# lijx10/DeepI2P

Measured on NVIDIA B200. Metric: registrations/sec, higher is better.
Workload: dtype f64

## Files before the change

deepi2p_b200/csrc/frustum_solver.cu:

```cuda
#include <cfloat>
#include <cmath>
#include <cstdarg>
#include <cstdlib>

#include "common.cuh"

namespace dib {

static thread_local char g_err[512] = "";
void set_error(const char* fmt, ...) {
  va_list ap;
  va_start(ap, fmt);
  vsnprintf(g_err, sizeof(g_err), fmt, ap);
  va_end(ap);
}

#ifndef DIB_WARPS_F4
#define DIB_WARPS_F4 10
#endif
#ifndef DIB_WARPS_F6
#define DIB_WARPS_F6 7
#endif
#ifndef DIB_WARPS_D4
#define DIB_WARPS_D4 7
#endif
#ifndef DIB_WARPS_D6
#define DIB_WARPS_D6 5
#endif
#ifndef DIB_CTAS_PER_SM
#define DIB_CTAS_PER_SM 2
#endif
template <typename CT, int P> struct Cfg;
template <> struct Cfg<float, 4> { static constexpr int kWarps = DIB_WARPS_F4; };
template <> struct Cfg<float, 6> { static constexpr int kWarps = DIB_WARPS_F6; };
template <> struct Cfg<double, 4> { static constexpr int kWarps = DIB_WARPS_D4; };
template <> struct Cfg<double, 6> { static constexpr int kWarps = DIB_WARPS_D6; };

struct Cam {
  double fx, fy, cx, cy, W1, H1, hW, hH;
};

struct PoseConst {
  double R[9];
  double t[3];
  double Jl[9];
  double cD, sD;
  int small;
};

template <int P>
struct NAcc {
  static constexpr int NA = P * (P + 1) / 2;
  static constexpr int N = 1 + P + NA;
};

__host__ __device__ constexpr int tri(int P, int j, int k) {
  return j * P - j * (j - 1) / 2 + (k - j);
}


template <int P>
__device__ __noinline__ void make_pose(const double* x, PoseConst* pc) {
  if (P == 4) {
    const double ry = x[0];
    pc->t[0] = x[1]; pc->t[1] = x[2]; pc->t[2] = x[3];
    double c, s;
    if (ry * ry > DBL_EPSILON) { sincos(ry, &s, &c); pc->cD = c; pc->sD = s; pc->small = 0; }
    else { c = 1.0; s = ry; pc->cD = 1.0; pc->sD = 0.0; pc->small = 1; }
    pc->R[0] = c; pc->R[1] = 0; pc->R[2] = s;
    pc->R[3] = 0; pc->R[4] = 1; pc->R[5] = 0;
    pc->R[6] = -s; pc->R[7] = 0; pc->R[8] = c;
  } else {
    const double ax = x[0], ay = x[1], az = x[2];
    pc->t[0] = x[3]; pc->t[1] = x[4]; pc->t[2] = x[5];
    const double th2 = ax * ax + ay * ay + az * az;
    if (th2 > DBL_EPSILON) {
      const double th = sqrt(th2);
      double s, c;
      sincos(th, &s, &c);
      const double wx = ax / th, wy = ay / th, wz = az / th;
      const double omc = 1.0 - c;
      pc->R[0] = c + wx * wx * omc;      pc->R[1] = wx * wy * omc - wz * s; pc->R[2] = wy * s + wx * wz * omc;
      pc->R[3] = wz * s + wx * wy * omc; pc->R[4] = c + wy * wy * omc;      pc->R[5] = -wx * s + wy * wz * omc;
      pc->R[6] = -wy * s + wx * wz * omc; pc->R[7] = wx * s + wy * wz * omc; pc->R[8] = c + wz * wz * omc;
      double sh, ch;
      sincos(0.5 * th, &sh, &ch);
      const double q = sh / (0.5 * th);
      const double A = 0.5 * q * q;
      double B;
      if (th < 0.5) {
        const double t2 = th2;
        B = 1.0 / 6.0 + t2 * (-1.0 / 120.0 + t2 * (1.0 / 5040.0 + t2 * (-1.0 / 362880.0 +
            t2 * (1.0 / 39916800.0 + t2 * (-1.0 / 6227020800.0 + t2 * (1.0 / 1307674368000.0))))));
      } else {
        B = (th - s) / (th2 * th);
      }
      pc->Jl[0] = 1.0 + B * (ax * ax - th2); pc->Jl[1] = -A * az + B * ax * ay;     pc->Jl[2] = A * ay + B * ax * az;
      pc->Jl[3] = A * az + B * ax * ay;      pc->Jl[4] = 1.0 + B * (ay * ay - th2); pc->Jl[5] = -A * ax + B * ay * az;
      pc->Jl[6] = -A * ay + B * ax * az;     pc->Jl[7] = A * ax + B * ay * az;      pc->Jl[8] = 1.0 + B * (az * az - th2);
      pc->small = 0;
    } else {
      pc->R[0] = 1;   pc->R[1] = -az; pc->R[2] = ay;
      pc->R[3] = az;  pc->R[4] = 1;   pc->R[5] = -ax;
      pc->R[6] = -ay; pc->R[7] = ax;  pc->R[8] = 1;
      for (int i = 0; i < 9; ++i) pc->Jl[i] = (i % 4 == 0) ? 1.0 : 0.0;
      pc->small = 1;
    }
    pc->cD = 0; pc->sD = 0;
  }
}

struct SmemAcc {
  double* base;
  __device__ __forceinline__ double& operator[](int j) const { return base[j * 32]; }
};

template <int P, typename ACC>
__device__ __forceinline__ void rank1(ACC acc, const double* J, double w, double r) {
  const double wr = w * r;
#pragma unroll
  for (int j = 0; j < P; ++j) {
    acc[1 + j] = fma(wr, J[j], acc[1 + j]);
    const double wj = w * J[j];
#pragma unroll
    for (int k = j; k < P; ++k) acc[1 + P + tri(P, j, k)] = fma(wj, J[k], acc[1 + P + tri(P, j, k)]);
  }
}

template <int P>
__device__ __forceinline__ bool point_rows(double px, double py, double pz, int lab, const Cam& cam,
                                           const PoseConst& pc, double r[3], double J[3][P], int* nrows) {
  constexpr int NR = P - 3;
  const double rx = fma(pc.R[0], px, fma(pc.R[1], py, pc.R[2] * pz));
  const double ry_ = fma(pc.R[3], px, fma(pc.R[4], py, pc.R[5] * pz));
  const double rz = fma(pc.R[6], px, fma(pc.R[7], py, pc.R[8] * pz));
  const double X = rx + pc.t[0], Y = ry_ + pc.t[1], Z = rz + pc.t[2];
  const double iz = 1.0 / Z;
  const double u = fma(cam.fx * X, iz, cam.cx);
  const double v = fma(cam.fy * Y, iz, cam.cy);

  bool any = false;
  double su = 0.0, sv = 0.0, sz = 0.0;
  if (lab == 0) {
    *nrows = 1;
    const double du_ = u - cam.hW, dv_ = v - cam.hH;
    const double xd = cam.hW - fabs(du_);
    const double yd = cam.hH - fabs(dv_);
    r[0] = 0.0;
    if (Z > 0.0 && xd > 0.0 && yd > 0.0) {
      r[0] = xd + yd;
      su = (du_ < 0.0) ? 1.0 : -1.0;
      sv = (dv_ < 0.0) ? 1.0 : -1.0;
      any = true;
    }
  } else {
    *nrows = 3;
    const double a0 = -u, b0 = u - cam.W1;
    const double a1 = -v, b1 = v - cam.H1;
    r[0] = (a0 < 0.0 ? 0.0 : a0) + (b0 < 0.0 ? 0.0 : b0);
    r[1] = (a1 < 0.0 ? 0.0 : a1) + (b1 < 0.0 ? 0.0 : b1);
    r[2] = (-Z < 0.0 ? 0.0 : -Z) * 100.0;
    su = (a0 < 0.0 ? 0.0 : -1.0) + (b0 < 0.0 ? 0.0 : 1.0);
    sv = (a1 < 0.0 ? 0.0 : -1.0) + (b1 < 0.0 ? 0.0 : 1.0);
    sz = (-Z < 0.0) ? 0.0 : -100.0;
    any = (su != 0.0) || (sv != 0.0) || (sz != 0.0);
  }
  if (!any) return false;

  double dX[NR], dY[NR], dZ[NR];
  if (P == 4) {
    dX[0] = fma(-pc.sD, px, pc.cD * pz);
    dY[0] = 0.0;
    dZ[0] = -fma(pc.cD, px, pc.sD * pz);
  } else {
    const double a = pc.small ? px : rx, b = pc.small ? py : ry_, c = pc.small ? pz : rz;
#pragma unroll
    for (int k = 0; k < 3; ++k) {
      dX[k] = c * pc.Jl[3 + k] - b * pc.Jl[6 + k];
      dY[k] = a * pc.Jl[6 + k] - c * pc.Jl[k];
      dZ[k] = b * pc.Jl[k] - a * pc.Jl[3 + k];
    }
  }
  const double au = cam.fx * iz, bu = (u - cam.cx) * iz;
  const double av = cam.fy * iz, bv = (v - cam.cy) * iz;
  double dU[P], dV[P];
#pragma unroll
  for (int k = 0; k < NR; ++k) {
    dU[k] = au * dX[k] - bu * dZ[k];
    dV[k] = av * dY[k] - bv * dZ[k];
  }
  dU[NR] = au; dU[NR + 1] = 0.0; dU[NR + 2] = -bu;
  dV[NR] = 0.0; dV[NR + 1] = av; dV[NR + 2] = -bv;
  if (lab == 0) {
#pragma unroll
    for (int j = 0; j < P; ++j) J[0][j] = su * dU[j] + sv * dV[j];
  } else {
#pragma unroll
    for (int j = 0; j < P; ++j) { J[0][j] = su * dU[j]; J[1][j] = sv * dV[j]; }
#pragma unroll
    for (int k = 0; k < NR; ++k) J[2][k] = sz * dZ[k];
    J[2][NR] = 0.0; J[2][NR + 1] = 0.0; J[2][NR + 2] = sz;
  }
  return true;
}

template <int P>
struct Proj {
  double X, Y, Z, iz, u, v;
  double dX[P - 3], dY[P - 3], dZ[P - 3];
};

template <int P>
__device__ __forceinline__ void project_point(double px, double py, double pz, bool valid, const Cam& cam,
                                              const PoseConst& pc, Proj<P>& o) {
  constexpr int NR = P - 3;
  if (!valid) { px = 0.0; py = 0.0; pz = 0.0; }
  double rx, ry_, rz;
  if (P == 4) {
    rx = fma(pc.R[0], px, pc.R[2] * pz);
    ry_ = py;
    rz = fma(pc.R[6], px, pc.R[8] * pz);
  } else {
    rx = fma(pc.R[0], px, fma(pc.R[1], py, pc.R[2] * pz));
    ry_ = fma(pc.R[3], px, fma(pc.R[4], py, pc.R[5] * pz));
    rz = fma(pc.R[6], px, fma(pc.R[7], py, pc.R[8] * pz));
  }
  o.X = rx + pc.t[0]; o.Y = ry_ + pc.t[1]; o.Z = rz + pc.t[2];
  const double zs = (valid && o.Z != 0.0) ? o.Z : 1.0;
  o.iz = 1.0 / zs;
  o.u = fma(cam.fx * o.X, o.iz, cam.cx);
  o.v = fma(cam.fy * o.Y, o.iz, cam.cy);
  if (P == 4) {
    o.dX[0] = fma(-pc.sD, px, pc.cD * pz);
    o.dY[0] = 0.0;
    o.dZ[0] = -fma(pc.cD, px, pc.sD * pz);
  } else {
    const double a = pc.small ? px : rx, b = pc.small ? py : ry_, c = pc.small ? pz : rz;
#pragma unroll
    for (int k = 0; k < NR; ++k) {
      o.dX[k] = c * pc.Jl[3 + k] - b * pc.Jl[6 + k];
      o.dY[k] = a * pc.Jl[6 + k] - c * pc.Jl[k];
      o.dZ[k] = b * pc.Jl[k] - a * pc.Jl[3 + k];
    }
  }
}

template <int P>
struct Out0 {
  double w, r, s1;
  double J[P];
};

template <int P>
__device__ __forceinline__ void eval_outside(double px, double py, double pz, bool valid, const Cam& cam,
                                             const PoseConst& pc, Out0<P>& o) {
  constexpr int NR = P - 3;
  Proj<P> q;
  project_point<P>(px, py, pz, valid, cam, pc, q);
  const double du_ = q.u - cam.hW, dv_ = q.v - cam.hH;
  const double xd = cam.hW - fabs(du_), yd = cam.hH - fabs(dv_);
  const bool act = valid && q.Z > 0.0 && xd > 0.0 && yd > 0.0;
  const double su = (du_ < 0.0) ? 1.0 : -1.0;
  const double sv = (dv_ < 0.0) ? 1.0 : -1.0;
  o.r = act ? xd + yd : 0.0;
  o.s1 = fma(o.r, o.r, 1.0);
  o.w = act ? 1.0 / o.s1 : 0.0;
  const double au = su * (cam.fx * q.iz), bu = su * ((q.u - cam.cx) * q.iz);
  const double av = sv * (cam.fy * q.iz), bv = sv * ((q.v - cam.cy) * q.iz);
#pragma unroll
  for (int k = 0; k < NR; ++k) {
    double j = au * q.dX[k] - (bu + bv) * q.dZ[k];
    if (P != 4) j = fma(av, q.dY[k], j);
    o.J[k] = j;
  }
  o.J[NR] = au; o.J[NR + 1] = av; o.J[NR + 2] = -(bu + bv);
}

template <int P>
struct Out1 {
  double w, r0, r1, r2, s1;
  double JU[P], JV[P], JZ[P];
};

template <int P>
__device__ __forceinline__ void eval_inside(double px, double py, double pz, bool valid, const Cam& cam,
                                            const PoseConst& pc, Out1<P>& o) {
  constexpr int NR = P - 3;
  Proj<P> q;
  project_point<P>(px, py, pz, valid, cam, pc, q);
  const double a0 = -q.u, b0 = q.u - cam.W1;
  const double a1 = -q.v, b1 = q.v - cam.H1;
  double su = (a0 < 0.0 ? 0.0 : -1.0) + (b0 < 0.0 ? 0.0 : 1.0);
  double sv = (a1 < 0.0 ? 0.0 : -1.0) + (b1 < 0.0 ? 0.0 : 1.0);
  double sz = (-q.Z < 0.0) ? 0.0 : -100.0;
  o.r0 = (a0 < 0.0 ? 0.0 : a0) + (b0 < 0.0 ? 0.0 : b0);
  o.r1 = (a1 < 0.0 ? 0.0 : a1) + (b1 < 0.0 ? 0.0 : b1);
  o.r2 = (-q.Z < 0.0 ? 0.0 : -q.Z) * 100.0;
  if (!valid) { su = 0.0; sv = 0.0; sz = 0.0; o.r0 = 0.0; o.r1 = 0.0; o.r2 = 0.0; }
  o.s1 = fma(o.r0, o.r0, fma(o.r1, o.r1, fma(o.r2, o.r2, 1.0)));
  o.w = 1.0 / o.s1;
  const double au = su * (cam.fx * q.iz), bu = su * ((q.u - cam.cx) * q.iz);
  const double av = sv * (cam.fy * q.iz), bv = sv * ((q.v - cam.cy) * q.iz);
#pragma unroll
  for (int k = 0; k < NR; ++k) {
    o.JU[k] = au * q.dX[k] - bu * q.dZ[k];
    o.JV[k] = (P == 4) ? -bv * q.dZ[k] : av * q.dY[k] - bv * q.dZ[k];
    o.JZ[k] = sz * q.dZ[k];
  }
  o.JU[NR] = au;  o.JU[NR + 1] = 0.0; o.JU[NR + 2] = -bu;
  o.JV[NR] = 0.0; o.JV[NR + 1] = av;  o.JV[NR + 2] = -bv;
  o.JZ[NR] = 0.0; o.JZ[NR + 1] = 0.0; o.JZ[NR + 2] = sz;
}

template <int P, unsigned MASK, typename ACC>
__device__ __forceinline__ void rank1_masked(ACC acc, const double* J, double w, double r) {
  const double wr = w * r;
#pragma unroll
  for (int j = 0; j < P; ++j) {
    if ((MASK >> j) & 1u) {
      acc[1 + j] = fma(wr, J[j], acc[1 + j]);
      const double wj = w * J[j];
#pragma unroll
      for (int k = j; k < P; ++k)
        if ((MASK >> k) & 1u) acc[1 + P + tri(P, j, k)] = fma(wj, J[k], acc[1 + P + tri(P, j, k)]);
    }
  }
}

template <int P, typename ACC>
__device__ __forceinline__ void accumulate_inside(ACC acc, const Out1<P>& o) {
  constexpr int NR = P - 3;
  constexpr unsigned ROT = (1u << NR) - 1u;
  rank1_masked<P, ROT | (1u << NR) | (1u << (NR + 2)), ACC>(acc, o.JU, o.w, o.r0);
  rank1_masked<P, ROT | (1u << (NR + 1)) | (1u << (NR + 2)), ACC>(acc, o.JV, o.w, o.r1);
  rank1_masked<P, ROT | (1u << (NR + 2)), ACC>(acc, o.JZ, o.w, o.r2);
}

__device__ __forceinline__ void renorm_product(double& prod, int& expo) {
  const int hi = __double2hiint(prod);
  const int e = ((hi >> 20) & 0x7ff) - 1023;
  if (e != 1024) {
    expo += e;
    prod = __hiloint2double(hi - (e << 20), __double2loint(prod));
  }
}

struct ClassConst {
  float zc[4], al[4], ah[4], bl[4], bh[4];
  float G, G0;
  int enabled;
};

__device__ __forceinline__ void make_class(const PoseConst& pc, const Cam& cam, ClassConst* cc, int lane) {
  const double gamma = 8.0 / 16777216.0;
  const int f = lane >> 2, j = lane & 3;
  double c = 0.0;
  if (lane < 20) {
    const double kx = (f == 1 || f == 2) ? cam.fx : 0.0;
    const double ky = (f >= 3) ? cam.fy : 0.0;
    const double kz = (f == 0) ? 1.0 : (f == 1) ? cam.cx : (f == 2) ? cam.cx - cam.W1 : (f == 3) ? cam.cy : cam.cy - cam.H1;
    const double a0 = (j < 3) ? pc.R[j] : pc.t[0];
    const double a1 = (j < 3) ? pc.R[3 + j] : pc.t[1];
    const double a2 = (j < 3) ? pc.R[6 + j] : pc.t[2];
    c = fma(kx, a0, fma(ky, a1, kz * a2));
  }
  const float cf = (float)c;
  if (lane < 20) cc->zc[lane] = cf;
  double amax = (lane < 20 && j < 3) ? fabs(c) : 0.0;
  double cmax = (lane < 20 && j == 3) ? fabs(c) : 0.0;
#pragma unroll
  for (int o = 16; o > 0; o >>= 1) {
    amax = fmax(amax, __shfl_xor_sync(0xffffffffu, amax, o));
    cmax = fmax(cmax, __shfl_xor_sync(0xffffffffu, cmax, o));
  }
  const bool finite = __all_sync(0xffffffffu, isfinite(cf));
  if (lane == 0) {
    cc->G = (float)(gamma * amax * 1.0000002);
    cc->G0 = (float)(gamma * cmax * 1.0000002) + 1e-30f;
    cc->enabled = (finite && isfinite(cc->G) && isfinite(cc->G0)) ? 1 : 0;
  }
}

template <int P>
__device__ __forceinline__ bool maybe_active(float x, float y, float z, int lab, const ClassConst& cc) {
  const bool lab_ok = (unsigned)lab <= 1u;
  const float m = fmaf(cc.G, fabsf(x) + fabsf(y) + fabsf(z), cc.G0);
  float Z, al, ah;
  if (P == 4) {
    Z = fmaf(cc.zc[0], x, fmaf(cc.zc[2], z, cc.zc[3]));
    al = fmaf(cc.al[0], x, fmaf(cc.al[2], z, cc.al[3]));
    ah = fmaf(cc.ah[0], x, fmaf(cc.ah[2], z, cc.ah[3]));
  } else {
    Z = fmaf(cc.zc[0], x, fmaf(cc.zc[1], y, fmaf(cc.zc[2], z, cc.zc[3])));
    al = fmaf(cc.al[0], x, fmaf(cc.al[1], y, fmaf(cc.al[2], z, cc.al[3])));
    ah = fmaf(cc.ah[0], x, fmaf(cc.ah[1], y, fmaf(cc.ah[2], z, cc.ah[3])));
  }
  const float bl = fmaf(cc.bl[0], x, fmaf(cc.bl[1], y, fmaf(cc.bl[2], z, cc.bl[3])));
  const float bh = fmaf(cc.bh[0], x, fmaf(cc.bh[1], y, fmaf(cc.bh[2], z, cc.bh[3])));
  const float lo4 = fminf(fminf(al, -ah), fminf(bl, -bh));
  const bool front = Z > m;
  const bool inside = front && lo4 > m;
  const bool outside = (Z < -m) || (front && lo4 < -m);
  const bool act = lab == 1 ? !inside : !outside;
  return lab_ok && (cc.enabled ? act : true);
}

constexpr int kBoxFields = 8;
constexpr int kRoundGroups = 32;
constexpr int kRoundPoints = kRoundGroups * 32;
constexpr int kBoxRoundFloats = kBoxFields * kRoundGroups;
#ifndef DIB_RING
#define DIB_RING 128
#endif
#ifndef DIB_GPS
#define DIB_GPS 2
#endif
#ifndef DIB_SLICE_ROUNDS
#define DIB_SLICE_ROUNDS 4
#endif
#ifndef DIB_SMALL_SLICE_ROUNDS
#define DIB_SMALL_SLICE_ROUNDS 2
#endif
#ifndef DIB_MAX_SLICES
#define DIB_MAX_SLICES 12
#endif
constexpr int kMaxSlices = DIB_MAX_SLICES;

__host__ __device__ inline int box_rounds(int n) { return (n + kRoundPoints - 1) / kRoundPoints; }
__host__ __device__ inline int slice_len(int rounds, int want) {
  int len = want < 1 ? 1 : want;
  const int need = (rounds + kMaxSlices - 1) / kMaxSlices;
  return len < need ? need : len;
}

template <typename CT> struct Entry;
template <> struct alignas(16) Entry<float> { float x, y, z; int lab; };
template <> struct alignas(16) Entry<double> { double x, y, z; long long lab; };

template <typename CT>
__global__ void __launch_bounds__(256) frustum_boxes_kernel(const CT* __restrict__ xyz,
                                                            const int8_t* __restrict__ label,
                                                            const int32_t* __restrict__ n_pts, int n_stride,
                                                            int rounds_max, float* __restrict__ table,
                                                            Entry<CT>* __restrict__ packed, int interleave) {
  const int s = blockIdx.y;
  const int lane = threadIdx.x & 31;
  const int gid = blockIdx.x * (blockDim.x >> 5) + (threadIdx.x >> 5);
  if (gid >= rounds_max * kRoundGroups) return;
  const int n = n_pts ? n_pts[s] : n_stride;
  int src = gid;
  if (interleave) {
    const int R = box_rounds(n);
    const int r = gid / kRoundGroups, q = gid % kRoundGroups;
    src = (r < R) ? q * R + r : rounds_max * kRoundGroups;
  }
  const int i_src = src * 32 + lane;
  const int i = gid * 32 + lane;
  double lo[3] = {1e300, 1e300, 1e300}, hi[3] = {-1e300, -1e300, -1e300};
  int lab = -1;
  Entry<CT> e;
  e.x = 0; e.y = 0; e.z = 0; e.lab = -1;
  if (i_src < n) {
    lab = label[(size_t)s * n_stride + i_src];
    if (lab == 0 || lab == 1) {
      e.x = xyz[((size_t)s * 3 + 0) * n_stride + i_src];
      e.y = xyz[((size_t)s * 3 + 1) * n_stride + i_src];
      e.z = xyz[((size_t)s * 3 + 2) * n_stride + i_src];
      e.lab = lab;
      lo[0] = hi[0] = (double)e.x; lo[1] = hi[1] = (double)e.y; lo[2] = hi[2] = (double)e.z;
    }
  }
  packed[(size_t)s * rounds_max * kRoundPoints + i] = e;
#pragma unroll
  for (int c = 0; c < 3; ++c)
#pragma unroll
    for (int o = 16; o > 0; o >>= 1) {
      lo[c] = fmin(lo[c], __shfl_xor_sync(0xffffffffu, lo[c], o));
      hi[c] = fmax(hi[c], __shfl_xor_sync(0xffffffffu, hi[c], o));
    }
  const unsigned m0 = __ballot_sync(0xffffffffu, lab == 0), m1 = __ballot_sync(0xffffffffu, lab == 1);
  if (lane == 0) {
    const int r = gid / kRoundGroups, q = gid % kRoundGroups;
    float* rec = table + ((size_t)s * rounds_max + r) * kBoxRoundFloats + q;
    const int flags = (m0 ? 1 : 0) | (m1 ? 2 : 0);
#pragma unroll
    for (int c = 0; c < 3; ++c) {
      float cf = 0.f, hf = 0.f;
      if (flags) {
        const double cd = 0.5 * (lo[c] + hi[c]);
        cf = (float)cd;
        const double hd = fmax(hi[c] - (double)cf, (double)cf - lo[c]);
        hf = (float)(hd * 1.000001 + (fabs(cd) + hd) * 1.3e-7 + 1e-30);
      }
      rec[c * kRoundGroups] = cf;
      rec[(3 + c) * kRoundGroups] = hf;
    }
    rec[6 * kRoundGroups] = __int_as_float(flags);
    rec[7 * kRoundGroups] = 0.f;
  }
}

struct LsSample {
  double x, value, gradient;
  int value_valid, gradient_valid;
};

template <int P>
struct LMState {
  static constexpr int NA = NAcc<P>::NA;
  double x[P], x_norm, cost, g[P], A[NA], grad_max;
  double scale[P], diag[P];
  double radius, dec;
  double step[P], delta[P], mcc;
  double lb[P], ub[P];
  double gd, dmax;
  LsSample lower, prev, cur;
  double xt[P];
  int reuse_diag, step_ok, invalid, iteration, max_iter;
  int phase;
  int ls_iter, evals, ls_steps, term;
};

constexpr int kBatch = 32;
constexpr int kRing = DIB_RING;
static_assert(kBatch + 32 * DIB_GPS <= kRing, "ring too small");

template <typename CT, int P>
struct WarpScratch {
  Entry<CT> ring[2][kRing];
  double accs[NAcc<P>::N][32];
};

template <typename CT, int P>
struct ProbCtx {
  double part[kMaxSlices][NAcc<P>::N];
  double tot[NAcc<P>::N];
  PoseConst pose;
  ClassConst cls;
  Cam cam;
  LMState<P> lm;
  const Entry<CT>* pk;
  const float* box;
  int rounds, slice_rounds, nslices;
  int len_full, nslices_full;
  int slice_after;
  int prob;
  int next_slice;
  int done;
};

template <typename CT, int P>
struct Smem {
  WarpScratch<CT, P> scratch[Cfg<CT, P>::kWarps];
  ProbCtx<CT, P> ctx[Cfg<CT, P>::kWarps];
  unsigned open_mask;
  int n_active;
};
static_assert(sizeof(Smem<float, 4>) * DIB_CTAS_PER_SM <= 227 * 1024, "4-DoF shared memory");
static_assert(sizeof(Smem<float, 6>) * DIB_CTAS_PER_SM <= 227 * 1024, "6-DoF shared memory");
static_assert(sizeof(Smem<double, 4>) * DIB_CTAS_PER_SM <= 227 * 1024, "4-DoF f64 shared memory");
static_assert(sizeof(Smem<double, 6>) * DIB_CTAS_PER_SM <= 227 * 1024, "6-DoF f64 shared memory");

struct BoxRec {
  float v[7];
};

__device__ __forceinline__ void box_load(const float* f, int slot, BoxRec& b) {
#pragma unroll
  for (int k = 0; k < 7; ++k) b.v[k] = __ldg(f + k * kRoundGroups + slot);
}

__device__ __forceinline__ int box_state(const BoxRec& b, const ClassConst& cc) {
  const int flags = __float_as_int(b.v[6]);
  if (flags == 0) return 0;
  if (!cc.enabled) return 1;
  const float cx = b.v[0], cy = b.v[1], cz = b.v[2], hx = b.v[3], hy = b.v[4], hz = b.v[5];
  const float m = 2.0f * fmaf(cc.G, (fabsf(cx) + hx) + (fabsf(cy) + hy) + (fabsf(cz) + hz), cc.G0);
  float lo[5], hi[5];
#pragma unroll
  for (int k = 0; k < 5; ++k) {
    const float* c = cc.zc + 4 * k;
    const float mid = fmaf(c[0], cx, fmaf(c[1], cy, fmaf(c[2], cz, c[3])));
    const float rad = fmaf(fabsf(c[0]), hx, fmaf(fabsf(c[1]), hy, fabsf(c[2]) * hz));
    lo[k] = mid - rad; hi[k] = mid + rad;
  }
  const bool front = lo[0] > m;
  const bool all_out = (hi[0] < -m) || (front && fminf(fminf(hi[1], -lo[2]), fminf(hi[3], -lo[4])) < -m);
  const bool all_in = front && fminf(fminf(lo[1], -hi[2]), fminf(lo[3], -hi[4])) > m;
  const bool skip = (!(flags & 1) || all_out) && (!(flags & 2) || all_in);
  if (skip) return 0;
  const bool sure = (flags == 1 && all_in) || (flags == 2 && all_out);
  return sure ? 2 : 1;
}

template <typename CT, int P>
__device__ __forceinline__ void eval_slice(WarpScratch<CT, P>& ws, const ProbCtx<CT, P>& pb, int r_begin, int r_end,
                                           double* part, int lane) {
  constexpr int N = NAcc<P>::N;
  const unsigned lt_mask = (1u << lane) - 1u;
  SmemAcc acc{&ws.accs[0][lane]};
#pragma unroll
  for (int j = 0; j < N; ++j) acc[j] = 0.0;
  const Cam& cam = pb.cam;
  const PoseConst& pc = pb.pose;
  const ClassConst& cc = pb.cls;
  const Entry<CT>* pk_s = pb.pk;
  const float* box_s = pb.box;
  Entry<CT>* ring0 = ws.ring[0];
  Entry<CT>* ring1 = ws.ring[1];
  int head0 = 0, pend0 = 0, head1 = 0, pend1 = 0;
  double prod = 1.0;
  int expo = 0;
  BoxRec box_cur, box_nxt;
#pragma unroll
  for (int k = 0; k < 7; ++k) { box_cur.v[k] = 0.f; box_nxt.v[k] = 0.f; }
  if (r_begin < r_end) box_load(box_s + (size_t)r_begin * kBoxRoundFloats, lane, box_nxt);

#pragma unroll 1
  for (int r = r_begin; r <= r_end; ++r) {
    unsigned mask = 0, mask_sure = 0;
    int threshold = 1;
    if (r < r_end) {
      threshold = kBatch;
      box_cur = box_nxt;
      if (r + 1 < r_end) box_load(box_s + (size_t)(r + 1) * kBoxRoundFloats, lane, box_nxt);
      const int bs = box_state(box_cur, cc);
      mask = __ballot_sync(0xffffffffu, bs == 1);
      mask_sure = __ballot_sync(0xffffffffu, bs == 2);
    }
    auto take_groups = [&](CT* lx, CT* ly, CT* lz, int* ll, bool& sure_only) -> bool {
      const bool any = (mask | mask_sure) != 0;
      sure_only = true;
      if (any) {
#pragma unroll
        for (int u = 0; u < DIB_GPS; ++u) {
          ll[u] = -1; lx[u] = 0; ly[u] = 0; lz[u] = 0;
          if (mask | mask_sure) {
            const bool from_sure = mask_sure != 0;
            const int b = __ffs(from_sure ? mask_sure : mask) - 1;
            if (from_sure) mask_sure &= mask_sure - 1; else mask &= mask - 1;
            sure_only = sure_only && from_sure;
            const Entry<CT> e = pk_s[(size_t)(r * kRoundGroups + b) * 32 + lane];
            ll[u] = (int)e.lab; lx[u] = e.x; ly[u] = e.y; lz[u] = e.z;
          }
        }
      }
      return any;
    };
#pragma unroll 1
    do {
      CT gx[DIB_GPS], gy[DIB_GPS], gz[DIB_GPS];
      int glab[DIB_GPS];
      bool all_sure = true;
      const bool have = take_groups(gx, gy, gz, glab, all_sure);
#pragma unroll 1
      while (pend0 >= threshold) {
        __syncwarp();
        const int take = pend0 < kBatch ? pend0 : kBatch;
        const Entry<CT> ea = ring0[(head0 + lane) & (kRing - 1)];
        Out0<P> oa;
        eval_outside<P>((double)ea.x, (double)ea.y, (double)ea.z, lane < take, cam, pc, oa);
        prod *= oa.s1;
        renorm_product(prod, expo);
        rank1<P, SmemAcc>(acc, oa.J, oa.w, oa.r);
        head0 = (head0 + take) & (kRing - 1);
        pend0 -= take;
      }
#pragma unroll 1
      while (pend1 >= threshold) {
        __syncwarp();
        const int take = pend1 < kBatch ? pend1 : kBatch;
        const Entry<CT> ea = ring1[(head1 + lane) & (kRing - 1)];
        Out1<P> oa;
        eval_inside<P>((double)ea.x, (double)ea.y, (double)ea.z, lane < take, cam, pc, oa);
        prod *= oa.s1;
        renorm_product(prod, expo);
        accumulate_inside<P, SmemAcc>(acc, oa);
        head1 = (head1 + take) & (kRing - 1);
        pend1 -= take;
      }
      if (have) {
        bool mb[DIB_GPS];
        if (all_sure) {
#pragma unroll
          for (int u = 0; u < DIB_GPS; ++u) mb[u] = (unsigned)glab[u] <= 1u;
        } else {
#pragma unroll
          for (int u = 0; u < DIB_GPS; ++u) mb[u] = maybe_active<P>((float)gx[u], (float)gy[u], (float)gz[u], glab[u], cc);
        }
#pragma unroll
        for (int u = 0; u < DIB_GPS; ++u) {
          const unsigned m1 = __ballot_sync(0xffffffffu, mb[u] && glab[u] == 1);
          const unsigned m0 = __ballot_sync(0xffffffffu, mb[u] && glab[u] == 0);
          if (mb[u]) {
            const bool l1 = glab[u] != 0;
            Entry<CT>* ring = l1 ? ring1 : ring0;
            const int at = (l1 ? head1 + pend1 : head0 + pend0) + __popc((l1 ? m1 : m0) & lt_mask);
            Entry<CT> e;
            e.x = gx[u]; e.y = gy[u]; e.z = gz[u]; e.lab = glab[u];
            ring[at & (kRing - 1)] = e;
          }
          pend0 += __popc(m0);
          pend1 += __popc(m1);
        }
      }
    } while (mask | mask_sure);
  }
  acc[0] = 0.5 * (log(prod) + (double)expo * 0.6931471805599453094);

  __syncwarp();
  if (lane < N) {
    double v = 0.0;
#pragma unroll 4
    for (int l = 0; l < 32; ++l) v += ws.accs[lane][(l + lane) & 31];
    part[lane] = v;
  }
  __syncwarp();
}

template <int P>
__device__ __forceinline__ void project_plus(const LMState<P>& st, const double* x, const double* d, double a, double* out) {
#pragma unroll
  for (int j = 0; j < P; ++j) {
    double v = fma(a, d[j], x[j]);
    v = fmax(v, st.lb[j]);
    v = fmin(v, st.ub[j]);
    out[j] = v;
  }
}

template <int P>
__device__ __forceinline__ double grad_max_norm(const LMState<P>& st, const double* x, const double* g) {
  double mx = 0.0;
#pragma unroll
  for (int j = 0; j < P; ++j) {
    double v = x[j] - g[j];
    v = fmax(v, st.lb[j]);
    v = fmin(v, st.ub[j]);
    mx = fmax(mx, fabs(x[j] - v));
  }
  return mx;
}

template <int P>
__device__ __forceinline__ bool chol_solve(const double (&As)[P][P], const double* d2, const double* gs, double* y) {
  double L[P][P], inv[P];
  bool ok = true;
#pragma unroll
  for (int j = 0; j < P; ++j) {
    double s = As[j][j] + d2[j];
#pragma unroll
    for (int k = 0; k < j; ++k) s = fma(-L[j][k], L[j][k], s);
    if (!(s > 0.0)) ok = false;
    inv[j] = rsqrt(s);
    L[j][j] = s * inv[j];
#pragma unroll
    for (int i = j + 1; i < P; ++i) {
      double t = As[i][j];
#pragma unroll
      for (int k = 0; k < j; ++k) t = fma(-L[i][k], L[j][k], t);
      L[i][j] = t * inv[j];
    }
  }
  double z[P];
#pragma unroll
  for (int i = 0; i < P; ++i) {
    double t = gs[i];
#pragma unroll
    for (int k = 0; k < i; ++k) t = fma(-L[i][k], z[k], t);
    z[i] = t * inv[i];
  }
#pragma unroll
  for (int i = P - 1; i >= 0; --i) {
    double t = z[i];
#pragma unroll
    for (int k = i + 1; k < P; ++k) t = fma(-L[k][i], y[k], t);
    y[i] = t * inv[i];
  }
  return ok;
}

constexpr unsigned kFull = 0xffffffffu;

__device__ __forceinline__ void durand_kerner_warp(const double (&c)[5], int deg, double (&roots)[4], int lane) {
  double radius = 0.0;
#pragma unroll
  for (int i = 1; i <= 4; ++i) {
    if (i <= deg) {
      const double a = fabs(c[i]) * (i == deg ? 0.5 : 1.0);
      radius = fmax(radius, a > 0.0 ? exp(log(a) / (double)i) : 0.0);
    }
  }
  radius = 2.0 * radius + 1e-300;
  const int me = lane % deg;
  double s, co;
  sincos(2.0 * 3.14159265358979323846 * me / deg + 0.4, &s, &co);
  double zr = 0.5 * radius * co, zi = 0.5 * radius * s;
#pragma unroll 1
  for (int it = 0; it < 100; ++it) {
    double nr = 0.0, ni = 0.0;
#pragma unroll
    for (int k = 0; k <= 4; ++k) {
      if (k <= deg) {
        const double tr = nr * zr - ni * zi + c[k];
        const double ti = nr * zi + ni * zr;
        nr = tr; ni = ti;
      }
    }
    double dr = 1.0, di = 0.0;
#pragma unroll
    for (int j = 0; j < 4; ++j) {
      if (j < deg) {
        const double zrj = __shfl_sync(kFull, zr, j), zij = __shfl_sync(kFull, zi, j);
        if (j != me) {
          const double er = zr - zrj, ei = zi - zij;
          const double tr = dr * er - di * ei, ti = dr * ei + di * er;
          dr = tr; di = ti;
        }
      }
    }
    double den = dr * dr + di * di;
    if (den == 0.0) { dr = 1e-300; di = 0.0; den = dr * dr; if (den == 0.0) den = 1e-300; }
    const double iden = 1.0 / den;
    const double qr = (nr * dr + ni * di) * iden, qi = (ni * dr - nr * di) * iden;
    zr -= qr; zi -= qi;
    double change = sqrt(qr * qr + qi * qi);
    change = fmax(change, __shfl_xor_sync(kFull, change, 1));
    change = fmax(change, __shfl_xor_sync(kFull, change, 2));
    if (change < 1e-14 * radius) break;
  }
#pragma unroll
  for (int i = 0; i < 4; ++i) roots[i] = __shfl_sync(kFull, zr, i);
}

__device__ __forceinline__ double mat_fetch(double e0, double e1, int i, int j) {
  const int src = ((i & 3) << 3) | j;
  const double v0 = __shfl_sync(kFull, e0, src), v1 = __shfl_sync(kFull, e1, src);
  return i < 4 ? v0 : v1;
}

__device__ __noinline__ double interp_min_step_warp(const LsSample& lower, const LsSample& previous, const LsSample& current,
                                                    double xmin, double xmax, int lane) {
  if (!current.value_valid) return fmin(fmax(current.x * 0.5, xmin), xmax);
  const LsSample* smp[3] = {&lower, &current, &previous};
  const int ns = previous.value_valid ? 3 : 2;
  int nc = 0;
#pragma unroll 1
  for (int i = 0; i < ns; ++i) { nc += smp[i]->value_valid ? 1 : 0; nc += smp[i]->gradient_valid ? 1 : 0; }
  const int deg = nc - 1;
  const int j = lane & 7, i0 = lane >> 3, i1 = 4 + (lane >> 3);
  auto element = [&](int r) -> double {
    if (r >= nc || j == 7) return 0.0;
    int row = 0, kind = -1;
    double sx = 0.0, rhs = 0.0;
#pragma unroll 1
    for (int i = 0; i < ns; ++i) {
      if (smp[i]->value_valid) { if (row == r) { sx = smp[i]->x; rhs = smp[i]->value; kind = 0; } ++row; }
      if (smp[i]->gradient_valid) { if (row == r) { sx = smp[i]->x; rhs = smp[i]->gradient; kind = 1; } ++row; }
    }
    if (j == 6) return rhs;
    const int e = (kind == 0) ? deg - j : deg - j - 1;
    if (e < 0) return 0.0;
    double pw = 1.0;
#pragma unroll 1
    for (int q = 0; q < e; ++q) pw = pw * sx;
    return (kind == 0) ? pw : (double)(e + 1) * pw;
  };
  double e0 = element(i0), e1 = (lane < 16) ? element(i1) : 0.0;

  unsigned perm = 0x543210u;
#pragma unroll 1
  for (int k = 0; k < nc; ++k) {
    double val = -1.0;
    int idx = 0x7fffffff;
    if (j >= k && j < nc) {
      if (i0 >= k && i0 < nc) { val = fabs(e0); idx = i0 * 8 + j; if (!(val > -1.0)) { val = -1.0; } }
      if (lane < 16 && i1 >= k && i1 < nc) {
        const double v1 = fabs(e1);
        if (v1 > val) { val = v1; idx = i1 * 8 + j; }
        else if (idx == 0x7fffffff) idx = i1 * 8 + j;
      }
    }
#pragma unroll
    for (int o = 1; o < 32; o <<= 1) {
      const double ov = __shfl_xor_sync(kFull, val, o);
      const int oi = __shfl_xor_sync(kFull, idx, o);
      if (ov > val || (ov == val && oi < idx)) { val = ov; idx = oi; }
    }
    if (val < 0.0) idx = k * 8 + k;
    if (val == 0.0) {
      if (j == 6) { if (i0 >= k && i0 < nc) e0 = 0.0; if (lane < 16 && i1 >= k && i1 < nc) e1 = 0.0; }
      break;
    }
    const int pr = idx >> 3, pcv = idx & 7;
    if (pr != k) {
      const double ak0 = mat_fetch(e0, e1, k, j), ap0 = mat_fetch(e0, e1, pr, j);
      if (i0 == k) e0 = ap0; else if (i0 == pr) e0 = ak0;
      if (i1 == k) e1 = ap0; else if (i1 == pr) e1 = ak0;
    }
    if (pcv != k) {
      const int jo = (j == k) ? pcv : ((j == pcv) ? k : j);
      const double n0 = __shfl_sync(kFull, e0, (i0 << 3) | jo), n1 = __shfl_sync(kFull, e1, (i0 << 3) | jo);
      e0 = n0; e1 = n1;
      const unsigned pa = (perm >> (4 * pcv)) & 15u, pb = (perm >> (4 * k)) & 15u;
      perm = (perm & ~((15u << (4 * pcv)) | (15u << (4 * k)))) | (pb << (4 * pcv)) | (pa << (4 * k));
    }
    const double pkk = mat_fetch(e0, e1, k, k);
    const double pkj = mat_fetch(e0, e1, k, j);
    const double a0 = __shfl_sync(kFull, e0, (i0 << 3) | k), a1 = __shfl_sync(kFull, e1, (i0 << 3) | k);
    if (j >= k && (j < nc || j == 6)) {
      if (i0 > k && i0 < nc) { const double f = a0 / pkk; e0 -= f * pkj; }
      if (lane < 16 && i1 > k && i1 < nc) { const double f = a1 / pkk; e1 -= f * pkj; }
    }
  }
  double zmine = 0.0;
#pragma unroll 1
  for (int k = nc - 1; k >= 0; --k) {
    const double mkk = mat_fetch(e0, e1, k, k);
    double sacc = mat_fetch(e0, e1, k, 6);
#pragma unroll 1
    for (int jj = k + 1; jj < nc; ++jj) sacc -= mat_fetch(e0, e1, k, jj) * __shfl_sync(kFull, zmine, jj);
    const double zk = (mkk == 0.0) ? 0.0 : sacc / mkk;
    if (lane == k) zmine = zk;
  }
  double pmine = 0.0;
#pragma unroll 1
  for (int k = 0; k < nc; ++k) {
    const double zk = __shfl_sync(kFull, zmine, k);
    if (lane == (int)((perm >> (4 * k)) & 15u)) pmine = zk;
  }
  auto poly_at = [&](double x) -> double {
    double v = 0.0;
#pragma unroll 1
    for (int i = 0; i < nc; ++i) v = v * x + __shfl_sync(kFull, pmine, i);
    return v;
  };
  double best_x = (xmin + xmax) / 2.0;
  double best_v = poly_at(best_x);
  const double vmin = poly_at(xmin);
  if (vmin < best_v) { best_v = vmin; best_x = xmin; }
  const double vmax = poly_at(xmax);
  if (vmax < best_v) { best_v = vmax; best_x = xmax; }
  if (nc <= 2) return best_x;
  const double dmine = (lane < deg) ? (double)(deg - lane) * pmine : 0.0;
  const unsigned zmask = __ballot_sync(kFull, lane < deg && dmine == 0.0);
  int lead = __ffs(~zmask) - 1;
  if (lead > deg) lead = deg;
  const double qmine = __shfl_sync(kFull, dmine, (lane + lead) & 31);
  const int rdeg = deg - lead - 1;
  double roots[4] = {0.0, 0.0, 0.0, 0.0};
  int nr = 0;
  if (rdeg == 1) {
    roots[0] = -__shfl_sync(kFull, qmine, 1) / __shfl_sync(kFull, qmine, 0);
    nr = 1;
  } else if (rdeg == 2) {
    const double a = __shfl_sync(kFull, qmine, 0), b = __shfl_sync(kFull, qmine, 1), c = __shfl_sync(kFull, qmine, 2);
    const double D = b * b - 4 * a * c;
    const double sD = sqrt(fabs(D));
    if (D >= 0) {
      if (b >= 0) { roots[0] = (-b - sD) / (2.0 * a); roots[1] = (2.0 * c) / (-b - sD); }
      else { roots[0] = (2.0 * c) / (-b + sD); roots[1] = (-b + sD) / (2.0 * a); }
    } else { roots[0] = -b / (2.0 * a); roots[1] = roots[0]; }
    nr = 2;
  } else if (rdeg >= 3) {
    const double ip0 = 1.0 / __shfl_sync(kFull, qmine, 0);
    double c[5];
#pragma unroll
    for (int i = 0; i < 5; ++i) c[i] = __shfl_sync(kFull, qmine, i) * ip0;
    durand_kerner_warp(c, rdeg, roots, lane);
    nr = rdeg;
  }
#pragma unroll
  for (int i = 0; i < 4; ++i) {
    if (i < nr && !(roots[i] < xmin || roots[i] > xmax)) {
      const double v = poly_at(roots[i]);
      if (v < best_v) { best_v = v; best_x = roots[i]; }
    }
  }
  return best_x;
}

enum { LM_DONE = 0, LM_EVAL = 1, LM_INTERP = 2 };

template <int P>
__device__ __noinline__ int lm_next_step(LMState<P>& st) {
  for (;;) {
    if (st.iteration >= st.max_iter) { st.term = 3; return LM_DONE; }
    if (st.step_ok && st.grad_max <= 1e-10) { st.term = 0; return LM_DONE; }
    if (st.radius <= 1e-32) { st.term = 4; return LM_DONE; }
    ++st.iteration;
    st.step_ok = 0;

    double As[P][P], gs[P], d2[P], y[P], sc[P];
#pragma unroll
    for (int j = 0; j < P; ++j) { sc[j] = st.scale[j]; gs[j] = st.g[j] * sc[j]; }
    {
      int idx = 0;
#pragma unroll
      for (int j = 0; j < P; ++j)
#pragma unroll
        for (int k = j; k < P; ++k) {
          const double v = st.A[idx++] * sc[j] * sc[k];
          As[j][k] = v; As[k][j] = v;
        }
    }
    if (!st.reuse_diag) {
#pragma unroll
      for (int j = 0; j < P; ++j) st.diag[j] = fmin(fmax(As[j][j], 1e-6), 1e32);
    }
    st.reuse_diag = 1;
    {
      const double inv_radius = 1.0 / st.radius;
#pragma unroll
      for (int j = 0; j < P; ++j) d2[j] = st.diag[j] * inv_radius;
    }
    bool ok = chol_solve<P>(As, d2, gs, y);
    double mcc = 0.0;
// ... 1036 lines not shown
```

Measured before the change: 6854.

## Store per-lane accumulators row-major and update them with double2 vector accesses

Moves the per-lane normal-equation accumulators in shared memory from a column-strided layout (one element per lane per row) to a per-lane contiguous row with padded stride. Updates now read and write pairs of entries with 128-bit double2 loads and stores, and the three inside-point rank-1 updates are fused into one pass over the row. The aim is to halve shared-memory instruction count and cut redundant load/store round trips. The cost is possible bank conflicts from the padded row layout and higher register pressure from the precomputed w*J arrays.

```diff
diff --git a/deepi2p_b200/csrc/frustum_solver.cu b/deepi2p_b200/csrc/frustum_solver.cu
--- a/deepi2p_b200/csrc/frustum_solver.cu
+++ b/deepi2p_b200/csrc/frustum_solver.cu
@@ -2,6 +2,7 @@
 #include <cmath>
 #include <cstdarg>
 #include <cstdlib>
+#include <utility>
 
 #include "common.cuh"
 
@@ -110,21 +111,66 @@
   }
 }
 
-struct SmemAcc {
-  double* base;
-  __device__ __forceinline__ double& operator[](int j) const { return base[j * 32]; }
+template <int P>
+struct AccRow {
+  static constexpr int N = NAcc<P>::N;
+  static constexpr int kPairs = (N + 1) / 2;
+  static constexpr int kStride = (2 * kPairs) % 4 == 0 ? 2 * kPairs + 2 : 2 * kPairs;
 };
 
-template <int P, typename ACC>
-__device__ __forceinline__ void rank1(ACC acc, const double* J, double w, double r) {
+__host__ __device__ constexpr int tri_row(int P, int t) {
+  int j = 0;
+  while (t >= P - j) { t -= P - j; ++j; }
+  return j;
+}
+
+template <int P, unsigned MASK, int A>
+struct AccTerm {
+  static constexpr bool kG = A >= 1 && A <= P;
+  static constexpr int kT = A - 1 - P;
+  static constexpr bool kH = A > P && A < NAcc<P>::N;
+  static constexpr int kJ = kG ? A - 1 : kH ? tri_row(P, kT) : 0;
+  static constexpr int kK = kH ? kJ + (kT - tri(P, kJ, kJ)) : 0;
+  static constexpr bool kHas = kG ? ((MASK >> kJ) & 1u) != 0 : kH && ((MASK >> kJ) & 1u) && ((MASK >> kK) & 1u);
+  static __device__ __forceinline__ double apply(double v, const double* J, double wr, const double* wJ) {
+    if (!kHas) return v;
+    return kG ? fma(wr, J[kJ], v) : fma(wJ[kJ], J[kK], v);
+  }
+};
+
+template <int P, typename F, int... I>
+__device__ __forceinline__ void for_pairs_impl(F&& f, std::integer_sequence<int, I...>) {
+  (f(std::integral_constant<int, I>{}), ...);
+}
+template <int P, typename F>
+__device__ __forceinline__ void for_pairs(F&& f) {
+  for_pairs_impl<P>(f, std::make_integer_sequence<int, AccRow<P>::kPairs>{});
+}
+
+template <int P>
+__device__ __forceinline__ void acc_zero(double* row) {
+#pragma unroll
+  for (int i = 0; i < AccRow<P>::kPairs; ++i) *reinterpret_cast<double2*>(row + 2 * i) = make_double2(0.0, 0.0);
+}
+
+template <int P>
+__device__ __forceinline__ void rank1(double* row, const double* J, double w, double r) {
+  constexpr unsigned ALL = (1u << P) - 1u;
   const double wr = w * r;
-#pragma unroll
-  for (int j = 0; j < P; ++j) {
-    acc[1 + j] = fma(wr, J[j], acc[1 + j]);
-    const double wj = w * J[j];
-#pragma unroll
-    for (int k = j; k < P; ++k) acc[1 + P + tri(P, j, k)] = fma(wj, J[k], acc[1 + P + tri(P, j, k)]);
-  }
+  double wJ[P];
+#pragma unroll
+  for (int j = 0; j < P; ++j) wJ[j] = w * J[j];
+  for_pairs<P>([&](auto ic) {
+    constexpr int a = 2 * decltype(ic)::value;
+    using T0 = AccTerm<P, ALL, a>;
+    using T1 = AccTerm<P, ALL, a + 1>;
+    if (T0::kHas || T1::kHas) {
+      double2 v = *reinterpret_cast<const double2*>(row + a);
+      v.x = T0::apply(v.x, J, wr, wJ);
+      v.y = T1::apply(v.y, J, wr, wJ);
+      *reinterpret_cast<double2*>(row + a) = v;
+    }
+  });
 }
 
 template <int P>
@@ -312,28 +358,28 @@
   o.JZ[NR] = 0.0; o.JZ[NR + 1] = 0.0; o.JZ[NR + 2] = sz;
 }
 
-template <int P, unsigned MASK, typename ACC>
-__device__ __forceinline__ void rank1_masked(ACC acc, const double* J, double w, double r) {
-  const double wr = w * r;
-#pragma unroll
-  for (int j = 0; j < P; ++j) {
-    if ((MASK >> j) & 1u) {
-      acc[1 + j] = fma(wr, J[j], acc[1 + j]);
-      const double wj = w * J[j];
-#pragma unroll
-      for (int k = j; k < P; ++k)
-        if ((MASK >> k) & 1u) acc[1 + P + tri(P, j, k)] = fma(wj, J[k], acc[1 + P + tri(P, j, k)]);
-    }
-  }
-}
-
-template <int P, typename ACC>
-__device__ __forceinline__ void accumulate_inside(ACC acc, const Out1<P>& o) {
+template <int P>
+__device__ __forceinline__ void accumulate_inside(double* row, const Out1<P>& o) {
   constexpr int NR = P - 3;
   constexpr unsigned ROT = (1u << NR) - 1u;
-  rank1_masked<P, ROT | (1u << NR) | (1u << (NR + 2)), ACC>(acc, o.JU, o.w, o.r0);
-  rank1_masked<P, ROT | (1u << (NR + 1)) | (1u << (NR + 2)), ACC>(acc, o.JV, o.w, o.r1);
-  rank1_masked<P, ROT | (1u << (NR + 2)), ACC>(acc, o.JZ, o.w, o.r2);
+  constexpr unsigned MU = ROT | (1u << NR) | (1u << (NR + 2));
+  constexpr unsigned MV = ROT | (1u << (NR + 1)) | (1u << (NR + 2));
+  constexpr unsigned MZ = ROT | (1u << (NR + 2));
+  const double wr0 = o.w * o.r0, wr1 = o.w * o.r1, wr2 = o.w * o.r2;
+  double wU[P], wV[P], wZ[P];
+#pragma unroll
+  for (int j = 0; j < P; ++j) { wU[j] = o.w * o.JU[j]; wV[j] = o.w * o.JV[j]; wZ[j] = o.w * o.JZ[j]; }
+  for_pairs<P>([&](auto ic) {
+    constexpr int a = 2 * decltype(ic)::value;
+    using U0 = AccTerm<P, MU, a>; using V0 = AccTerm<P, MV, a>; using Z0 = AccTerm<P, MZ, a>;
+    using U1 = AccTerm<P, MU, a + 1>; using V1 = AccTerm<P, MV, a + 1>; using Z1 = AccTerm<P, MZ, a + 1>;
+    if (U0::kHas || V0::kHas || Z0::kHas || U1::kHas || V1::kHas || Z1::kHas) {
+      double2 v = *reinterpret_cast<const double2*>(row + a);
+      v.x = Z0::apply(V0::apply(U0::apply(v.x, o.JU, wr0, wU), o.JV, wr1, wV), o.JZ, wr2, wZ);
+      v.y = Z1::apply(V1::apply(U1::apply(v.y, o.JU, wr0, wU), o.JV, wr1, wV), o.JZ, wr2, wZ);
+      *reinterpret_cast<double2*>(row + a) = v;
+    }
+  });
 }
 
 __device__ __forceinline__ void renorm_product(double& prod, int& expo) {
@@ -528,7 +574,7 @@
 template <typename CT, int P>
 struct WarpScratch {
   Entry<CT> ring[2][kRing];
-  double accs[NAcc<P>::N][32];
+  double accs[32][AccRow<P>::kStride];
 };
 
 template <typename CT, int P>
@@ -598,9 +644,8 @@
                                            double* part, int lane) {
   constexpr int N = NAcc<P>::N;
   const unsigned lt_mask = (1u << lane) - 1u;
-  SmemAcc acc{&ws.accs[0][lane]};
-#pragma unroll
-  for (int j = 0; j < N; ++j) acc[j] = 0.0;
+  double* acc = &ws.accs[lane][0];
+  acc_zero<P>(acc);
   const Cam& cam = pb.cam;
   const PoseConst& pc = pb.pose;
   const ClassConst& cc = pb.cls;
@@ -662,7 +707,7 @@
         eval_outside<P>((double)ea.x, (double)ea.y, (double)ea.z, lane < take, cam, pc, oa);
         prod *= oa.s1;
         renorm_product(prod, expo);
-        rank1<P, SmemAcc>(acc, oa.J, oa.w, oa.r);
+        rank1<P>(acc, oa.J, oa.w, oa.r);
         head0 = (head0 + take) & (kRing - 1);
         pend0 -= take;
       }
@@ -675,7 +720,7 @@
         eval_inside<P>((double)ea.x, (double)ea.y, (double)ea.z, lane < take, cam, pc, oa);
         prod *= oa.s1;
         renorm_product(prod, expo);
-        accumulate_inside<P, SmemAcc>(acc, oa);
+        accumulate_inside<P>(acc, oa);
         head1 = (head1 + take) & (kRing - 1);
         pend1 -= take;
       }
@@ -712,7 +757,7 @@
   if (lane < N) {
     double v = 0.0;
 #pragma unroll 4
-    for (int l = 0; l < 32; ++l) v += ws.accs[lane][(l + lane) & 31];
+    for (int l = 0; l < 32; ++l) v += ws.accs[(l + lane) & 31][lane];
     part[lane] = v;
   }
   __syncwarp();
```

Result: no change. 6814, median of 6 (-0.6%).
